# LuoGuiwen/MSM_blst

Measured on AMD Instinct MI355X. Metric: G1 MSM point-scalar pairs/sec at n=2^20, 1/2/4/8 MI355X; bit-exact vs CPU, higher is better.
Workload: dtype u32 (exact Fp381 integer arithmetic, 14x28-bit limbs)

## Files before the change

include/msm_mi355x.h:

```cpp
#ifndef MSM_MI355X_H
#define MSM_MI355X_H

#include <stddef.h>
#include <stdint.h>

#ifdef __cplusplus
extern "C" {
#endif

typedef uint8_t byte;
typedef uint64_t limb_t;
typedef struct { byte b[256 / 8]; } blst_scalar;
typedef struct { limb_t l[384 / 8 / sizeof(limb_t)]; } blst_fp;
typedef struct { blst_fp fp[2]; } blst_fp2;
typedef struct { blst_fp x, y, z; } blst_p1;
typedef struct { blst_fp x, y; } blst_p1_affine;
typedef struct { blst_fp2 x, y, z; } blst_p2;
typedef struct { blst_fp2 x, y; } blst_p2_affine;
typedef struct { blst_fp x, y, zzz, zz; } blst_p1xyzz;
typedef struct { blst_fp2 x, y, zzz, zz; } blst_p2xyzz;
typedef struct { int m; int b; int alpha; } digit_decomposition;

size_t blst_p1s_mult_pippenger_scratch_sizeof(size_t npoints);
void blst_p1s_mult_pippenger(blst_p1 *ret, const blst_p1_affine *const points[], size_t npoints,
// ... 222 lines not shown
void msm_gen_scalars(byte *out32, size_t n, uint64_t seed);
void msm_p1_fixed_points(blst_p1_affine *out, size_t n);
void msm_p2_fixed_points(blst_p2_affine *out, size_t n);
void msm_p1_fixed_points_range(blst_p1_affine *out, size_t start, size_t n);
void msm_p2_fixed_points_range(blst_p2_affine *out, size_t start, size_t n);
void msm_p1_to_affine(blst_p1_affine *out, const blst_p1 *in);
void msm_p2_to_affine(blst_p2_affine *out, const blst_p2 *in);
void msm_p1_compress(byte out[48], const blst_p1 *in);
void msm_p2_compress(byte out[96], const blst_p2 *in);
void msm_p1_add(blst_p1 *out, const blst_p1 *a, const blst_p1 *b);
void msm_p2_add(blst_p2 *out, const blst_p2 *a, const blst_p2 *b);

int msm_test_field(int group, int op, const limb_t *a, const limb_t *b, limb_t *out, size_t n);
int msm_test_xyzz(int group, const void *points_affine, size_t npoints, const uint32_t *ops, int len, size_t nseq,
                  void *out);

#ifdef __cplusplus
}
#endif
#endif
```

msm_blst_amd/_ffi.py:

```python
import ctypes
import os

HERE = os.path.dirname(os.path.abspath(__file__))
LIB_PATH = os.path.join(HERE, "libmsm_mi355x.so")

_lib = None


class MsmError(RuntimeError):
    pass


def lib():
    global _lib
    if _lib is not None:
        return _lib
    if not os.path.exists(LIB_PATH):
        raise MsmError(f"{LIB_PATH} not built: run `python -m msm_blst_amd.build` (hipcc, gfx950)")
    L = ctypes.CDLL(LIB_PATH)
    vp, sz, i32, u64 = ctypes.c_void_p, ctypes.c_size_t, ctypes.c_int, ctypes.c_uint64
    for g in (1, 2):
        f = getattr(L, f"blst_p{g}s_mult_pippenger")
        f.argtypes = [vp, vp, sz, vp, sz, vp]
        f.restype = None
# ... 9 lines not shown
            getattr(L, name).argtypes = [vp, vp]
        getattr(L, f"msm_p{g}_add").argtypes = [vp, vp, vp]
    L.msm_last_error.restype = ctypes.c_char_p
    L.msm_device_count.restype = i32
    L.msm_ctx_create.argtypes = [ctypes.POINTER(vp), i32, i32, i32]
    L.msm_ctx_set_points.argtypes = [vp, vp, sz, i32, vp]
    L.msm_ctx_mult.argtypes = [vp, vp, vp, sz, sz, i32, vp]
    L.msm_ctx_mult_batch.argtypes = [vp, vp, vp, sz, sz, sz, sz, i32, vp]
    L.msm_ctx_set_profiling.argtypes = [vp, i32]
    L.msm_ctx_phase_times.argtypes = [vp, vp]
    L.msm_ctx_destroy.argtypes = [vp]
    L.msm_ctx_destroy.restype = None
    L.msm_gen_scalars.argtypes = [vp, sz, u64]
    L.msm_test_field.argtypes = [i32, i32, vp, vp, vp, sz]
    L.msm_test_xyzz.argtypes = [i32, vp, sz, vp, i32, sz, vp]
    pp = ctypes.POINTER(vp)
    L.msm_ches_params.argtypes = [i32, i32, vp]
    L.msm_ches_ctx_create.argtypes = [pp, i32, i32, i32, i32]
    L.msm_ches_ctx_create_params.argtypes = [pp, i32, i32, vp]
    L.msm_ches_ctx_create_multi.argtypes = [pp, i32, vp, i32, i32, i32]
    L.msm_ches_ctx_shards.argtypes = [vp]
    L.msm_ches_ctx_build_table.argtypes = [vp, vp, sz, i32, vp]
    L.msm_ches_ctx_set_table.argtypes = [vp, vp, sz, i32, vp]
    L.msm_ches_ctx_get_table.argtypes = [vp, vp, sz, sz]
    L.msm_ches_ctx_mult.argtypes = [vp, vp, vp, sz, i32, vp]
    L.msm_ches_ctx_mult_batch.argtypes = [vp, vp, vp, sz, sz, sz, i32, vp]
    L.msm_ches_ctx_set_profiling.argtypes = [vp, i32]
    L.msm_ches_ctx_phase_times.argtypes = [vp, vp]
    L.msm_ches_ctx_bucket_count.argtypes = [vp]
    L.msm_ches_ctx_bucket_count.restype = sz
# ... 84 lines not shown
```

msm_blst_amd/csrc/abi.cpp:

```cpp
#include <hip/hip_runtime.h>
#include <stdio.h>
#include <stdlib.h>
#include <string.h>

#include <algorithm>
#include <atomic>
#include <map>
#include <memory>
#include <mutex>
#include <string>

#include "../../include/msm_mi355x.h"
#include "decode.hpp"
#include "encode.hpp"
#include "engine.hpp"
#include "hash_to_curve.hpp"
#include "multi.hpp"
#include "pairing.hpp"
#include "point_segments.hpp"
#include "points_mult.hpp"
#include "pool.hpp"
#include "ptr_walk.hpp"
#include "table_registry.hpp"
#include "to_affine.hpp"
// ... 1645 lines not shown
    return MSM_OK;
  } catch (const std::exception &e) {
    return fail(MSM_E_HIP, e.what());
  }
}
int msm_test_xyzz(int group, const void *pts, size_t npts, const uint32_t *ops, int len, size_t nseq, void *out) {
  try {
    if (group == 1) test_xyzz<1>((const uint64_t *)pts, npts, ops, len, nseq, (uint64_t *)out);
    else test_xyzz<2>((const uint64_t *)pts, npts, ops, len, nseq, (uint64_t *)out);
    return MSM_OK;
  } catch (const std::exception &e) {
    return fail(MSM_E_HIP, e.what());
  }
}

#define WB_DISPATCH(ctx, CALL) ((ctx)->group == 1 ? (ctx)->g1->CALL : (ctx)->g2->CALL)

int msm_wbits_ctx_create(msm_wbits_ctx **ctx, int group, int device, int wbits) {
  if (!ctx || (group != 1 && group != 2)) return fail(MSM_E_ARG, "bad ctx/group");
  if (msm_device_count() <= device || device < 0) return fail(MSM_E_NODEV, "no such HIP device");
  try {
    auto c = std::make_unique<msm_wbits_ctx>();
    c->group = group;
    c->device = device;
    if (group == 1) c->g1 = std::make_unique<Wbits<1>>(device, wbits);
    else c->g2 = std::make_unique<Wbits<2>>(device, wbits);
    *ctx = c.release();
    return MSM_OK;
  } catch (const std::exception &e) {
    return fail(MSM_E_ARG, e.what());
// ... 74 lines not shown
```

msm_blst_amd/csrc/bucket_sort.hpp:

```cpp
#pragma once
#include <hip/hip_runtime.h>
#include <stdint.h>

namespace msm {

constexpr int BS_TILE = 4096;
constexpr int BS_MAX_FB_BITS = 12;
constexpr int BS_MAX_CB = 8192;
constexpr uint32_t BS_NONE = 0xffffffffu;
constexpr int SCHED_PER_THREAD = 16;
constexpr int SCHED_PER_BLOCK = 256 * SCHED_PER_THREAD;
__device__ __forceinline__ uint32_t sched_class(uint32_t c) { return 255u - (c < 255u ? c : 255u); }

static __global__ void __launch_bounds__(256)
    k_bs_hist(const uint32_t *__restrict__ keys, size_t ne, int fb_bits, int ncb, int ntiles,
              uint32_t *__restrict__ ghist, uint32_t *__restrict__ classes) {
  __shared__ uint32_t h[BS_MAX_CB];
  keys += (size_t)blockIdx.y * ne;
  ghist += (size_t)blockIdx.y * ncb * ntiles;
  if (blockIdx.x == 0)
    for (int c = threadIdx.x; c < 512; c += blockDim.x) classes[(size_t)blockIdx.y * 512 + c] = 0;
  for (int b = threadIdx.x; b < ncb; b += blockDim.x) h[b] = 0;
  __syncthreads();
  const size_t t0 = (size_t)blockIdx.x * BS_TILE;
  uint32_t kk[BS_TILE / 256];
#pragma unroll
  for (int r = 0; r < BS_TILE / 256; ++r) {
    size_t e = t0 + threadIdx.x + (size_t)r * 256;
    kk[r] = e < ne ? keys[e] : BS_NONE;
  }
#pragma unroll
  for (int r = 0; r < BS_TILE / 256; ++r)
    if (kk[r] != BS_NONE) atomicAdd(&h[kk[r] >> fb_bits], 1u);
  __syncthreads();
  for (int b = threadIdx.x; b < ncb; b += blockDim.x) ghist[(size_t)b * ntiles + blockIdx.x] = h[b];
}

__device__ __forceinline__ uint32_t block_exclusive_scan_256(uint32_t *a, int n, uint32_t *wsum) {
  const int t = threadIdx.x, lane = t & 63, wave = t >> 6;
  const int per = (n + 255) / 256, lo = t * per, hi = min(n, lo + per);
  uint32_t s = 0;
  for (int i = lo; i < hi; ++i) s += a[i];
  uint32_t incl = s;
#pragma unroll
  for (int d = 1; d < 64; d <<= 1) {
    uint32_t v = __shfl_up(incl, d, 64);
    if (lane >= d) incl += v;
  }
  if (lane == 63) wsum[wave] = incl;
  __syncthreads();
// ... 92 lines not shown
    int i = t * per + k;
    if (k < per && i < n) a[i] = base + loc[k];
  }
  __syncthreads();
}

constexpr int BS_FINE_CAP = 30 * 1024;
constexpr int BS_FINE_STEP = BS_FINE_CAP - BS_FINE_CAP / 8;
constexpr int BS_FINE_MAXW = 8;

template <int BT>
static __global__ void __launch_bounds__(BT)
    k_bs_fine(const uint32_t *__restrict__ okeys, const uint32_t *__restrict__ ovals, int fb_bits, int ncb,
              int ntiles, const uint32_t *__restrict__ gbase, const uint32_t *__restrict__ ghist, uint32_t nb,
              uint32_t *__restrict__ sorted, uint32_t *__restrict__ counts, uint32_t *__restrict__ offsets,
              uint32_t *__restrict__ class_total, int nsets) {
  __shared__ uint32_t off[1 << BS_MAX_FB_BITS];
  __shared__ uint8_t win[1 << BS_MAX_FB_BITS];
  __shared__ uint32_t stage[BS_FINE_CAP];
  __shared__ uint32_t wsum[BT / 64];
  __shared__ uint32_t wb[BS_FINE_MAXW + 1];
  __shared__ uint32_t cls[256];
  const int FB = 1 << fb_bits;
  const uint32_t fmask = (uint32_t)FB - 1u;
  const int b = blockIdx.x, set = blockIdx.y;
  const size_t per = (size_t)ncb * ntiles, s0 = (size_t)set * per;
  const size_t last = (size_t)nsets * per - 1;
  const uint32_t lo = gbase[s0 + (size_t)b * ntiles];
  const uint32_t hi = b + 1 < ncb ? gbase[s0 + (size_t)(b + 1) * ntiles]
                                  : (set + 1 < nsets ? gbase[s0 + per] : gbase[last] + ghist[last]);
  counts += (size_t)set * nb;
  offsets += (size_t)set * nb;
  class_total += (size_t)set * 512;
  const uint32_t nbin = hi - lo;
  for (int f = threadIdx.x; f < FB; f += blockDim.x) off[f] = 0;
  for (int c = threadIdx.x; c < 256; c += BT) cls[c] = 0;
  if (threadIdx.x <= BS_FINE_MAXW) wb[threadIdx.x] = nbin;
  __syncthreads();
  constexpr int U = 16, UW = 12;
  for (uint32_t e0 = lo; e0 < hi; e0 += U * BT) {
    uint32_t kk[U];
#pragma unroll
    for (int r = 0; r < U; ++r) {
      uint32_t e = e0 + threadIdx.x + r * BT;
      kk[r] = e < hi ? okeys[e] : BS_NONE;
    }
#pragma unroll
    for (int r = 0; r < U; ++r)
      if (kk[r] != BS_NONE) atomicAdd(&off[kk[r] & fmask], 1u);
// ... 59 lines not shown
        if (kk[r] == BS_NONE || win[kk[r] & fmask] != k) continue;
        uint32_t li = atomicAdd(&off[kk[r] & fmask], 1u) - base;
        if (li < (uint32_t)BS_FINE_CAP)
          stage[li] = vv[r];
        else
          sorted[lo + base + li] = vv[r];
      }
    }
    __syncthreads();
    const uint32_t nst = min(end - base, (uint32_t)BS_FINE_CAP);
    for (uint32_t i = threadIdx.x; i < nst; i += BT) sorted[lo + base + i] = stage[i];
    __syncthreads();
  }
}

static __global__ void __launch_bounds__(256, 6)
    k_sched_scatter(const uint32_t *__restrict__ counts, const uint32_t *__restrict__ offsets, uint32_t nb,
                    uint32_t *__restrict__ class_total, uint32_t *__restrict__ order, uint32_t *__restrict__ scnt,
                    uint32_t *__restrict__ soff) {
  __shared__ uint32_t h[256];
  __shared__ uint32_t base[256];
  __shared__ uint32_t wsum[4];
  counts += (size_t)blockIdx.y * nb;
  offsets += (size_t)blockIdx.y * nb;
  order += (size_t)blockIdx.y * nb;
  scnt += (size_t)blockIdx.y * nb;
  soff += (size_t)blockIdx.y * nb;
  class_total += (size_t)blockIdx.y * 512;
  const uint32_t t = threadIdx.x, b0 = blockIdx.x * SCHED_PER_BLOCK, lane = t & 63, wave = t >> 6;
  h[t] = 0;
  const uint32_t v = class_total[t];
  uint32_t incl = v;
#pragma unroll
  for (int d = 1; d < 64; d <<= 1) {
    uint32_t u = __shfl_up(incl, d, 64);
    if (lane >= (uint32_t)d) incl += u;
  }
  if (lane == 63) wsum[wave] = incl;
  __syncthreads();
  uint32_t cbase = incl - v;
  for (uint32_t w = 0; w < wave; ++w) cbase += wsum[w];
  uint32_t rank[SCHED_PER_THREAD], cnt[SCHED_PER_THREAD];
#pragma unroll
  for (int r = 0; r < SCHED_PER_THREAD; ++r) {
    const uint32_t b = b0 + r * 256 + t;
    cnt[r] = b < nb ? counts[b] : 0u;
    rank[r] = b < nb ? atomicAdd(&h[sched_class(cnt[r])], 1u) : 0u;
  }
  __syncthreads();
  if (h[t]) base[t] = cbase + atomicAdd(&class_total[256 + t], h[t]);
  __syncthreads();
#pragma unroll
  for (int r = 0; r < SCHED_PER_THREAD; ++r) {
    const uint32_t b = b0 + r * 256 + t;
    if (b < nb) {
      const uint32_t pos = base[sched_class(cnt[r])] + rank[r];
      order[pos] = b;
      scnt[pos] = cnt[r];
      soff[pos] = offsets[b];
    }
  }
}

constexpr size_t BS_IPAY_SLACK = 64 * 256;
static __global__ void __launch_bounds__(256)
    k_interleave(const uint32_t *__restrict__ scnt, const uint32_t *__restrict__ soff, uint32_t nb, uint32_t nw,
                 const uint32_t *__restrict__ class_total, const uint32_t *__restrict__ sorted,
                 uint32_t *__restrict__ ipay, size_t ipay_stride, uint32_t *__restrict__ wbase) {
  __shared__ uint32_t ct[256], hs[256], wsum[4];
  const size_t set = blockIdx.y;
  const uint32_t t = threadIdx.x, lane = t & 63, wave = t >> 6;
  const uint32_t tot = class_total[set * 512 + t];
  uint32_t incl = tot;
// ... 53 lines not shown
```

msm_blst_amd/csrc/ches.hip:

```cpp
#include <hipcub/hipcub.hpp>

#include <algorithm>
#include <cstdlib>
#include <cstring>

#include "ches_kernels.hpp"
#include "coop.hpp"
#include "engine.hpp"
#include "hoststage.hpp"
#include "pair_kernels.hpp"

#ifndef MSM_GROUP
#error "define MSM_GROUP (1 or 2)"
#endif

namespace msm {

#if MSM_GROUP == 1
static const ChesParams kChesTable[] = {
    {8, 0, 12, 22, 7, 6, 857, 10, 26},         {9, 0, 13, 20, 231, 6, 1725, 11, 24},
    {10, 0, 13, 20, 231, 6, 1725, 12, 22},     {11, 0, 14, 19, 7, 6, 3417, 13, 20},
    {12, 0, 14, 19, 7, 6, 3417, 13, 20},       {13, 0, 16, 16, 29677, 6, 18343, 15, 17},
    {14, 0, 16, 16, 29677, 6, 18343, 15, 17},  {15, 0, 16, 16, 29677, 6, 18343, 16, 16},
    {16, 0, 19, 14, 231, 6, 109244, 17, 15},   {16, 1, 18, 15, 7, 6, 54618, 17, 15},
// ... 732 lines not shown
  f.counts.ensure(NB * nsets * 4);
  f.offsets.ensure(NB * nsets * 4);
  f.order.ensure(NB * nsets * 4);
  static const bool fused_env = [] {
    const char *e = getenv("MSM_FRONT_FUSED");
    return !e || atoi(e) != 0;
  }();
  if (fused_env && (p_.h == 12 || p_.h == 13 || p_.h == 14 || p_.h == 16 || p_.h == 19 || p_.h == 20)) {
    const int ntiles = (int)nblk(n, 256);
    const BucketSort::Geom g = f.sort.prepare(s, ne, (uint32_t)NB, nsets, ntiles);
#define MSM_CHES_FRONT(HT)                                                                                             \
  do {                                                                                                                 \
    hipLaunchKernelGGL(k_ches_front_hist<HT>, dim3(ntiles, nsets), dim3(256), 0, s, d_scalars, stride, n, p_.q_exp,   \
                       code_.as<uint32_t>(), rank_.as<uint2>(), (uint32_t)B_.size(), (uint32_t)small_,                 \
                       (uint32_t)copies_, set_stride, g.fb_bits, g.ncb, g.ntiles, f.sort.ghist.as<uint32_t>(),         \
                       f.sort.classes.as<uint32_t>());                                                                  \
    MSM_HIP_CHECK(hipGetLastError());                                                                                  \
    if (profile_) MSM_HIP_CHECK(hipEventRecord(ev_[1], s));                                                            \
    f.sort.scan(s, g);                                                                                                 \
    hipLaunchKernelGGL(k_ches_front_coarse<HT>, dim3(ntiles, nsets), dim3(256), (size_t)(2 * g.ncb + 512 * HT) * 4, s, \
                       d_scalars, stride, n, p_.q_exp, code_.as<uint32_t>(), rank_.as<uint2>(), (uint32_t)B_.size(),  \
                       (uint32_t)small_, (uint32_t)copies_, set_stride, g.fb_bits, g.ncb, g.ntiles,                   \
                       f.sort.gbase.as<uint32_t>(), f.sort.okeys.as<uint32_t>(), f.sort.ovals.as<uint32_t>());         \
    MSM_HIP_CHECK(hipGetLastError());                                                                                  \
  } while (0)
    switch (p_.h) {
      case 12: MSM_CHES_FRONT(12); break;
      case 13: MSM_CHES_FRONT(13); break;
      case 14: MSM_CHES_FRONT(14); break;
      case 16: MSM_CHES_FRONT(16); break;
      case 19: MSM_CHES_FRONT(19); break;
// ... 220 lines not shown
  }
  auto group_tail = [&](hipStream_t ts, int rset, size_t first, size_t nmsm, bool last_group) {
    if (bit_tail && last_group) {
      red.launch_tail_group_bits(ts, rset, (int)nmsm, tail_coop);
      red.copy_out_group_bits(ts, rset, (int)nmsm, host_bits_);
    } else {
      red.launch_tail_group(ts, rset, (int)nmsm, tail_coop && last_group);
      red.copy_out_group(ts, rset, (int)nmsm, out_base + first * ob);
    }
  };
  static const size_t fg_env = [] {
    const char *e = getenv("MSM_FRONT_GROUP");
    return e ? (size_t)std::min(kFrontGroup, std::max(1, atoi(e))) : (size_t)0;
  }();
  const int nl = batch_lanes();
  static const int fine_bt = [] {
    const char *e = getenv("MSM_FINE_BT");
    return e && atoi(e) == 256 ? 256 : 1024;
  }();
  static const bool acc_group_env = [] {
    const char *e = getenv("MSM_ACC_GROUP");
    return !e || atoi(e) != 0;
  }();
  const bool acc_groups = nl >= 2 && nseg == 1 && acc_group_env;
  const size_t fg_max = !packed ? 1 : fg_env ? fg_env : acc_groups ? 4 : nl >= 3 ? 4 : nl == 2 ? 2 : (size_t)kFrontGroupDefault;
  const std::vector<size_t> fgb = front_groups(count, fg_max);
  const size_t nfg = fgb.size() - 1;
  const size_t NB = bucket_count(), n = n_;
  if (acc_groups)
    for (DevBuf &b : gbuckets_) b.ensure(fg_max * NB * sizeof(Xyzz<typename FieldOf<G>::F>));
  else
    for (int b = 0; b < std::max(kBSets, nl); ++b) buckets_[b].ensure(NB * sizeof(Xyzz<typename FieldOf<G>::F>));
  static const bool phase_env = [] {
    const char *e = getenv("MSM_FRONT_PHASE");
// ... 286 lines not shown
```

msm_blst_amd/csrc/ches_kernels.hpp:

```cpp
#pragma once
#include "bucket_sort.hpp"
#include "kernels.hpp"

namespace msm {

constexpr uint32_t CH_IDX_MASK = 0x00ffffffu;

__device__ constexpr uint64_t PM2[6] = {0xb9feffffffffaaa9ull, 0x1eabfffeb153ffffull, 0x6730d2a0f6b0f624ull,
                                        0x64774b84f38512bfull, 0x4b1ba7b6434bacd7ull, 0x1a0111ea397fe69aull};
__device__ __forceinline__ void fp_inv(Fp &r, const Fp &a) {
  Fp a1 = a, a2, a3, acc;
  fp_norm(a1);
  fp_sqr(a2, a1);
  fp_mul(a3, a2, a1);
  fp_one(acc);
  for (int k = 190; k >= 0; --k) {
    if (k != 190) {
      fp_sqr(acc, acc);
      fp_sqr(acc, acc);
    }
    const uint32_t w = (uint32_t)(PM2[k >> 5] >> ((k & 31) * 2)) & 3u;
    if (w) {
      const uint32_t m1 = 0u - (uint32_t)(w == 1), m2 = 0u - (uint32_t)(w == 2), m3 = 0u - (uint32_t)(w == 3);
      Fp t;
// ... 270 lines not shown
    }
    if (j == HT - 1 && b != 0 && b <= small) {
      const uint32_t cp = (uint32_t)(i % copies);
      if (cp) b = nb0 + (cp - 1) * small + b - 1;
    }
    key[j] = b ? b : KEY_NONE;
    val[j] = (uint32_t)(3 * (i * (size_t)HT + j) + (c & 3u)) | ((c & 4u) << 29);
  }
}

template <int HT>
static __global__ void __launch_bounds__(256)
    k_ches_front_hist(const uint8_t *__restrict__ scalars, size_t stride, size_t n, int q_exp,
                      const uint32_t *__restrict__ code, const uint2 *__restrict__ rank, uint32_t nb0, uint32_t small,
                      uint32_t copies, size_t set_stride, int fb_bits, int ncb, int ntiles, uint32_t *__restrict__ ghist,
                      uint32_t *__restrict__ classes) {
  __shared__ uint32_t h[BS_MAX_CB];
  scalars += (size_t)blockIdx.y * set_stride;
  ghist += (size_t)blockIdx.y * ncb * ntiles;
  if (blockIdx.x == 0)
    for (int c = threadIdx.x; c < 512; c += blockDim.x) classes[(size_t)blockIdx.y * 512 + c] = 0;
  for (int b = threadIdx.x; b < ncb; b += blockDim.x) h[b] = 0;
  __syncthreads();
  const size_t i = (size_t)blockIdx.x * blockDim.x + threadIdx.x;
  if (i < n) {
    uint32_t key[HT], val[HT];
    ches_entries<HT>(scalars + i * stride, stride, i, q_exp, code, rank, nb0, small, copies, key, val);
#pragma unroll
    for (int j = 0; j < HT; ++j)
      if (key[j] != KEY_NONE) atomicAdd(&h[key[j] >> fb_bits], 1u);
  }
  __syncthreads();
  for (int b = threadIdx.x; b < ncb; b += blockDim.x) ghist[(size_t)b * ntiles + blockIdx.x] = h[b];
}

template <int HT>
static __global__ void __launch_bounds__(256)
    k_ches_front_coarse(const uint8_t *__restrict__ scalars, size_t stride, size_t n, int q_exp,
                        const uint32_t *__restrict__ code, const uint2 *__restrict__ rank, uint32_t nb0,
                        uint32_t small, uint32_t copies, size_t set_stride, int fb_bits, int ncb, int ntiles,
                        const uint32_t *__restrict__ gbase, uint32_t *__restrict__ okeys,
                        uint32_t *__restrict__ ovals) {
  extern __shared__ uint32_t sm[];
  __shared__ uint32_t wsum[4];
  uint32_t *loff = sm, *gb = sm + ncb, *sk = sm + 2 * ncb, *sv = sk + 256 * HT;
  scalars += (size_t)blockIdx.y * set_stride;
  gbase += (size_t)blockIdx.y * ncb * ntiles;
  for (int b = threadIdx.x; b < ncb; b += blockDim.x) {
    loff[b] = 0;
    gb[b] = gbase[(size_t)b * ntiles + blockIdx.x];
  }
  __syncthreads();
  const size_t i = (size_t)blockIdx.x * blockDim.x + threadIdx.x;
  uint32_t key[HT], val[HT], rk[HT];
  if (i < n) {
    ches_entries<HT>(scalars + i * stride, stride, i, q_exp, code, rank, nb0, small, copies, key, val);
  } else {
#pragma unroll
    for (int j = 0; j < HT; ++j) key[j] = KEY_NONE, val[j] = 0;
  }
#pragma unroll
  for (int j = 0; j < HT; ++j) rk[j] = key[j] != KEY_NONE ? atomicAdd(&loff[key[j] >> fb_bits], 1u) : 0u;
  __syncthreads();
  const uint32_t total = block_exclusive_scan_256(loff, ncb, wsum);
#pragma unroll
  for (int j = 0; j < HT; ++j) {
    if (key[j] == KEY_NONE) continue;
    const uint32_t pos = loff[key[j] >> fb_bits] + rk[j];
    sk[pos] = key[j];
    sv[pos] = val[j];
  }
  __syncthreads();
  for (uint32_t e = threadIdx.x; e < total; e += 256) {
    const uint32_t k = sk[e], b = k >> fb_bits;
    const uint32_t g = gb[b] + (e - loff[b]);
    okeys[g] = k;
    ovals[g] = sv[e];
  }
}

__device__ __forceinline__ void r_minus(uint32_t s[8]) {
  int64_t br = 0;
#pragma unroll
  for (int k = 0; k < 8; ++k) {
    int64_t d = (int64_t)FR_R32[k] - (int64_t)s[k] + br;
// ... 183 lines not shown
```

msm_blst_amd/csrc/engine.hip:

```cpp
#include <hipcub/hipcub.hpp>

#include <algorithm>

#include "bucket_sort.hpp"
#include "engine.hpp"
#include "hoststage.hpp"
#include "kernels.hpp"
#include "pair_kernels.hpp"

#ifndef MSM_GROUP
#error "define MSM_GROUP (1 or 2)"
#endif

namespace msm {

#if MSM_GROUP == 1
BucketSort::Geom BucketSort::prepare(hipStream_t s, size_t ne, uint32_t nb, int nsets, int ntiles) {
  Geom g;
  g.fb_bits = 8;
  while (g.fb_bits < BS_MAX_FB_BITS && ((size_t)nb >> g.fb_bits) > 384) ++g.fb_bits;
  g.ncb = (int)(((size_t)nb + (1u << g.fb_bits) - 1) >> g.fb_bits);
  if (g.ncb > BS_MAX_CB || g.ncb > 4096) throw std::runtime_error("BucketSort: too many buckets");
  if (nsets < 1 || nsets > 65535) throw std::runtime_error("BucketSort: bad set count");
  if (ne * nsets >= (1ull << 32)) throw std::runtime_error("BucketSort: too many entries");
  g.ntiles = ntiles > 0 ? ntiles : (int)std::max<size_t>(1, (ne + BS_TILE - 1) / BS_TILE);
  g.nslots = (size_t)nsets * g.ncb * g.ntiles;
  if (g.nslots >= (1ull << 31)) throw std::runtime_error("BucketSort: too many histogram slots");
  ghist.ensure(g.nslots * 4);
  gbase.ensure(g.nslots * 4);
  okeys.ensure(std::max<size_t>(ne * nsets, 1) * 4);
  ovals.ensure(std::max<size_t>(ne * nsets, 1) * 4);
  wbase.ensure(groups(nb) * nsets * 4);
  ipay_stride = ne + BS_IPAY_SLACK;
  ipay.ensure(ipay_stride * nsets * 4);
  size_t scan_tmp = 0;
  hipcub::DeviceScan::ExclusiveSum(nullptr, scan_tmp, ghist.as<uint32_t>(), gbase.as<uint32_t>(), (int)g.nslots, s);
  tmp.ensure(scan_tmp);
  g.scan_tmp = scan_tmp;
  classes.ensure((size_t)512 * 4 * nsets);
  scnt.ensure((size_t)nb * nsets * 4);
  soff.ensure((size_t)nb * nsets * 4);
  return g;
}

void BucketSort::scan(hipStream_t s, const Geom &g) {
  size_t tb = g.scan_tmp;
  MSM_HIP_CHECK(
      hipcub::DeviceScan::ExclusiveSum(tmp.p, tb, ghist.as<uint32_t>(), gbase.as<uint32_t>(), (int)g.nslots, s));
}

void BucketSort::run(hipStream_t s, const uint32_t *keys, const uint32_t *vals, size_t ne, uint32_t nb,
                     uint32_t *sorted, uint32_t *counts, uint32_t *offsets, uint32_t *order, int nsets) {
  const Geom g = prepare(s, ne, nb, nsets, 0);
  hipLaunchKernelGGL(k_bs_hist, dim3(g.ntiles, nsets), dim3(256), 0, s, keys, ne, g.fb_bits, g.ncb, g.ntiles,
                     ghist.as<uint32_t>(), classes.as<uint32_t>());
  MSM_HIP_CHECK(hipGetLastError());
  scan(s, g);
  hipLaunchKernelGGL(k_bs_coarse, dim3(g.ntiles, nsets), dim3(256), (size_t)(2 * g.ncb + 2 * BS_TILE) * 4, s, keys,
                     vals, ne, g.fb_bits, g.ncb, g.ntiles, gbase.as<uint32_t>(), okeys.as<uint32_t>(),
                     ovals.as<uint32_t>());
  MSM_HIP_CHECK(hipGetLastError());
  finish(s, g, ne, nb, sorted, counts, offsets, order, nsets);
}

void BucketSort::finish(hipStream_t s, const Geom &g, size_t ne, uint32_t nb, uint32_t *sorted, uint32_t *counts,
                        uint32_t *offsets, uint32_t *order, int nsets) {
  (void)ne;
  const int fb_bits = g.fb_bits, ncb = g.ncb, ntiles = g.ntiles;
  const size_t nw = groups(nb);
  if (fine_bt == 256)
    hipLaunchKernelGGL(k_bs_fine<256>, dim3(ncb, nsets), dim3(256), 0, s, okeys.as<uint32_t>(),
                       ovals.as<uint32_t>(), fb_bits, ncb, ntiles, gbase.as<uint32_t>(), ghist.as<uint32_t>(), nb,
                       sorted, counts, offsets, classes.as<uint32_t>(), nsets);
  else
    hipLaunchKernelGGL(k_bs_fine<1024>, dim3(ncb, nsets), dim3(1024), 0, s, okeys.as<uint32_t>(),
                       ovals.as<uint32_t>(), fb_bits, ncb, ntiles, gbase.as<uint32_t>(), ghist.as<uint32_t>(), nb,
                       sorted, counts, offsets, classes.as<uint32_t>(), nsets);
  MSM_HIP_CHECK(hipGetLastError());
  hipLaunchKernelGGL(k_sched_scatter, dim3(nblk(nb, SCHED_PER_BLOCK), nsets), dim3(256), 0, s, counts, offsets, nb,
                     classes.as<uint32_t>(), order, scnt.as<uint32_t>(), soff.as<uint32_t>());
  MSM_HIP_CHECK(hipGetLastError());
  hipLaunchKernelGGL(k_interleave, dim3((unsigned)nw / 4 + 1, nsets), dim3(256), 0, s, scnt.as<uint32_t>(),
                     soff.as<uint32_t>(), nb, (uint32_t)nw, classes.as<uint32_t>(), sorted, ipay.as<uint32_t>(),
                     ipay_stride, wbase.as<uint32_t>());
  MSM_HIP_CHECK(hipGetLastError());
}
#endif


template <int G>
Pippenger<G>::Pippenger(int device, int window_bits) : dev_(device), c_(window_bits) {
  if (c_ < 8 || c_ > 20) throw std::runtime_error("window_bits out of range [8,20]");
// ... 514 lines not shown
```

msm_blst_amd/csrc/engine.hpp:

```cpp
#pragma once
#include <hip/hip_runtime.h>
#include <stdint.h>

#include <cstdlib>
#include <memory>
#include <stdexcept>
#include <string>
#include <vector>

#include "acc_sched.hpp"
#include "host_fp.hpp"

#define MSM_HIP_CHECK(x)                                                                           \
  do {                                                                                            \
    hipError_t e_ = (x);                                                                          \
    if (e_ != hipSuccess)                                                                         \
      throw std::runtime_error(std::string("HIP error ") + hipGetErrorString(e_) + " at " + #x); \
  } while (0)

namespace msm {

class HostStager;

inline unsigned nblk(size_t n, unsigned b) { return (unsigned)((n + b - 1) / b); }
// ... 50 lines not shown
  int accumulate_launches = 0;
};

template <int G>
struct HostField;
template <>
struct HostField<1> {
  typedef hfp::Fp F;
};
template <>
struct HostField<2> {
  typedef hfp::Fp2 F;
};

struct BucketSort {
  DevBuf ghist, gbase, okeys, ovals, classes, tmp;
  DevBuf scnt, soff, wbase, ipay;
  size_t ipay_stride = 0;
  int fine_bt = 1024;
  static size_t groups(size_t nb) { return (nb + 63) / 64; }
  AccSched sched(const uint32_t *order, const uint32_t *sorted, size_t set, size_t nb) const {
    const size_t nw = groups(nb);
    return AccSched{order + set * nb,
                    scnt.as<uint32_t>() + set * nb,
                    soff.as<uint32_t>() + set * nb,
                    wbase.as<uint32_t>() + set * nw,
                    ipay.as<uint32_t>() + set * ipay_stride,
                    sorted};
  }
  AccStride stride(size_t nb) const { return AccStride{nb, groups(nb), ipay_stride}; }
  void run(hipStream_t s, const uint32_t *keys, const uint32_t *vals, size_t ne, uint32_t nb, uint32_t *sorted,
           uint32_t *counts, uint32_t *offsets, uint32_t *order, int nsets = 1);
  struct Geom {
    int fb_bits = 8, ncb = 1, ntiles = 1;
    size_t nslots = 0, scan_tmp = 0;
  };
  Geom prepare(hipStream_t s, size_t ne, uint32_t nb, int nsets, int ntiles);
  void scan(hipStream_t s, const Geom &g);
  void finish(hipStream_t s, const Geom &g, size_t ne, uint32_t nb, uint32_t *sorted, uint32_t *counts,
              uint32_t *offsets, uint32_t *order, int nsets);
  size_t device_bytes() const {
    return ghist.bytes + gbase.bytes + okeys.bytes + ovals.bytes + classes.bytes + tmp.bytes + scnt.bytes + soff.bytes +
           wbase.bytes + ipay.bytes;
  }
};

template <class HF>
hfp::Jac<HF> horner(const std::vector<hfp::Jac<HF>> &T, int c) {
  hfp::Jac<HF> ret = T.back();
  for (int w = (int)T.size() - 2; w >= 0; --w) {
    for (int k = 0; k < c; ++k) ret = hfp::dbl(ret);
    ret = hfp::addj(ret, T[w]);
  }
  return ret;
}


// ... 314 lines not shown
```

Baseline: 459.4 million.

## Replace hipcub scan with fused bin-total scan and add split fine-sort kernel

Drops the hipcub DeviceScan over the histogram. The histogram kernels now atomically accumulate per-bin totals, and a custom k_bs_scan kernel derives each bin's base from those totals and scans its tiles, so no temp buffer or multi-pass library scan is needed. The fine kernel resets bin_total so it can be reused on the next call. The change also adds an optional split fine-sort kernel, selected only via MSM_FINE_BT=split, compacts registers in the front-sort and sched-scatter kernels by packing rank and class bits, and adds a test entry point. The risks are atomic contention on bin_total and the quadratic prefix sum that each scan block does over earlier bins.

New measurement: 457.8 million. About the same (-0.3%).

```diff
diff --git a/include/msm_mi355x.h b/include/msm_mi355x.h
--- a/include/msm_mi355x.h
+++ b/include/msm_mi355x.h
@@ -260,6 +260,10 @@
 int msm_test_field(int group, int op, const limb_t *a, const limb_t *b, limb_t *out, size_t n);
 int msm_test_xyzz(int group, const void *points_affine, size_t npoints, const uint32_t *ops, int len, size_t nseq,
                   void *out);
+int msm_test_bucket_sort(int device, const uint32_t *d_keys, const uint32_t *d_vals, size_t ne, uint32_t nb, int nsets,
+                         int fine, uint32_t *counts, uint32_t *offsets, uint32_t *sorted, uint32_t *order,
+                         uint32_t *scnt, uint32_t *soff, uint32_t *wbase, uint32_t *ipay, uint32_t *ghist,
+                         uint32_t *gbase, size_t geom[4]);
 
 #ifdef __cplusplus
 }
diff --git a/msm_blst_amd/_ffi.py b/msm_blst_amd/_ffi.py
--- a/msm_blst_amd/_ffi.py
+++ b/msm_blst_amd/_ffi.py
@@ -47,6 +47,8 @@
     L.msm_gen_scalars.argtypes = [vp, sz, u64]
     L.msm_test_field.argtypes = [i32, i32, vp, vp, vp, sz]
     L.msm_test_xyzz.argtypes = [i32, vp, sz, vp, i32, sz, vp]
+    if hasattr(L, "msm_test_bucket_sort"):
+        L.msm_test_bucket_sort.argtypes = [i32, vp, vp, sz, ctypes.c_uint32, i32, i32] + [vp] * 11
     pp = ctypes.POINTER(vp)
     L.msm_ches_params.argtypes = [i32, i32, vp]
     L.msm_ches_ctx_create.argtypes = [pp, i32, i32, i32, i32]
diff --git a/msm_blst_amd/csrc/abi.cpp b/msm_blst_amd/csrc/abi.cpp
--- a/msm_blst_amd/csrc/abi.cpp
+++ b/msm_blst_amd/csrc/abi.cpp
@@ -1683,6 +1683,48 @@
   }
 }
 
+int msm_test_bucket_sort(int device, const uint32_t *d_keys, const uint32_t *d_vals, size_t ne, uint32_t nb, int nsets,
+                         int fine, uint32_t *counts, uint32_t *offsets, uint32_t *sorted, uint32_t *order,
+                         uint32_t *scnt, uint32_t *soff, uint32_t *wbase, uint32_t *ipay, uint32_t *ghist,
+                         uint32_t *gbase, size_t geom[4]) {
+  if (!d_keys || !d_vals || !ne || !nb || nsets < 1 || (fine != 1024 && fine != 256 && fine != BucketSort::FINE_SPLIT))
+    return fail(MSM_E_ARG, "bad args");
+  if (msm_device_count() <= device || device < 0) return fail(MSM_E_NODEV, "no such HIP device");
+  try {
+    DeviceGuard dg(device);
+    BucketSort bs;
+    bs.fine_bt = fine;
+    DevBuf d_sorted, d_counts, d_offsets, d_order;
+    const size_t nbs = (size_t)nb * nsets * 4;
+    d_sorted.ensure(ne * nsets * 4 + 64);
+    d_counts.ensure(nbs);
+    d_offsets.ensure(nbs);
+    d_order.ensure(nbs);
+    hipStream_t s = nullptr;
+    bs.run(s, d_keys, d_vals, ne, nb, d_sorted.as<uint32_t>(), d_counts.as<uint32_t>(), d_offsets.as<uint32_t>(),
+           d_order.as<uint32_t>(), nsets);
+    const BucketSort::Geom g = bs.prepare(s, ne, nb, nsets, 0);
+    MSM_HIP_CHECK(hipStreamSynchronize(s));
+    auto get = [&](uint32_t *dst, const void *src, size_t bytes) {
+      if (dst) MSM_HIP_CHECK(hipMemcpy(dst, src, bytes, hipMemcpyDeviceToHost));
+    };
+    get(counts, d_counts.p, nbs);
+    get(offsets, d_offsets.p, nbs);
+    get(order, d_order.p, nbs);
+    get(sorted, d_sorted.p, ne * nsets * 4);
+    get(scnt, bs.scnt.p, nbs);
+    get(soff, bs.soff.p, nbs);
+    get(wbase, bs.wbase.p, BucketSort::groups(nb) * nsets * 4);
+    get(ipay, bs.ipay.p, bs.ipay_stride * nsets * 4);
+    get(ghist, bs.ghist.p, g.nslots * 4);
+    get(gbase, bs.gbase.p, g.nslots * 4);
+    if (geom) geom[0] = (size_t)g.fb_bits, geom[1] = (size_t)g.ncb, geom[2] = (size_t)g.ntiles, geom[3] = bs.ipay_stride;
+    return MSM_OK;
+  } catch (const std::exception &e) {
+    return fail(MSM_E_HIP, e.what());
+  }
+}
+
 #define WB_DISPATCH(ctx, CALL) ((ctx)->group == 1 ? (ctx)->g1->CALL : (ctx)->g2->CALL)
 
 int msm_wbits_ctx_create(msm_wbits_ctx **ctx, int group, int device, int wbits) {
diff --git a/msm_blst_amd/csrc/bucket_sort.hpp b/msm_blst_amd/csrc/bucket_sort.hpp
--- a/msm_blst_amd/csrc/bucket_sort.hpp
+++ b/msm_blst_amd/csrc/bucket_sort.hpp
@@ -12,9 +12,15 @@
 constexpr int SCHED_PER_BLOCK = 256 * SCHED_PER_THREAD;
 __device__ __forceinline__ uint32_t sched_class(uint32_t c) { return 255u - (c < 255u ? c : 255u); }
 
+constexpr int FRONT_ACC_WAVES = 3;
+constexpr int front_vgpr_alloc(int vgprs) { return (vgprs + 7) / 8 * 8; }
+constexpr int front_vgpr_free(int acc_vgprs) { return 512 - FRONT_ACC_WAVES * front_vgpr_alloc(acc_vgprs); }
+constexpr int FRONT_MAX_THREADS = 256;
+constexpr int FRONT_MAX_LDS = 80 * 1024;
+
 static __global__ void __launch_bounds__(256)
     k_bs_hist(const uint32_t *__restrict__ keys, size_t ne, int fb_bits, int ncb, int ntiles,
-              uint32_t *__restrict__ ghist, uint32_t *__restrict__ classes) {
+              uint32_t *__restrict__ ghist, uint32_t *__restrict__ classes, uint32_t *__restrict__ bin_total) {
   __shared__ uint32_t h[BS_MAX_CB];
   keys += (size_t)blockIdx.y * ne;
   ghist += (size_t)blockIdx.y * ncb * ntiles;
@@ -33,7 +39,61 @@
   for (int r = 0; r < BS_TILE / 256; ++r)
     if (kk[r] != BS_NONE) atomicAdd(&h[kk[r] >> fb_bits], 1u);
   __syncthreads();
-  for (int b = threadIdx.x; b < ncb; b += blockDim.x) ghist[(size_t)b * ntiles + blockIdx.x] = h[b];
+  bin_total += (size_t)blockIdx.y * ncb;
+  for (int b = threadIdx.x; b < ncb; b += blockDim.x) {
+    ghist[(size_t)b * ntiles + blockIdx.x] = h[b];
+    if (h[b]) atomicAdd(&bin_total[b], h[b]);
+  }
+}
+
+static __global__ void __launch_bounds__(256)
+    k_bs_scan(const uint32_t *__restrict__ ghist, const uint32_t *__restrict__ bin_total, int ncb, int ntiles,
+              uint32_t *__restrict__ gbase) {
+  __shared__ uint32_t wsum[4];
+  const int t = threadIdx.x, lane = t & 63, wave = t >> 6;
+  const size_t slot = (size_t)blockIdx.y * ncb + blockIdx.x;
+  uint32_t s = 0;
+  for (size_t i = t; i < slot; i += 256) s += bin_total[i];
+#pragma unroll
+  for (int d = 32; d; d >>= 1) s += __shfl_xor(s, d, 64);
+  if (lane == 0) wsum[wave] = s;
+  __syncthreads();
+  uint32_t run = wsum[0] + wsum[1] + wsum[2] + wsum[3];
+  __syncthreads();
+  ghist += slot * ntiles;
+  gbase += slot * ntiles;
+  constexpr int PER = 4;
+  for (int c0 = 0; c0 < ntiles; c0 += 256 * PER) {
+    const int i0 = c0 + t * PER;
+    uint32_t x[PER], sum = 0;
+#pragma unroll
+    for (int k = 0; k < PER; ++k) {
+      x[k] = i0 + k < ntiles ? ghist[i0 + k] : 0u;
+      sum += x[k];
+    }
+    uint32_t incl = sum;
+#pragma unroll
+    for (int d = 1; d < 64; d <<= 1) {
+      uint32_t v = __shfl_up(incl, d, 64);
+      if (lane >= d) incl += v;
+    }
+    if (lane == 63) wsum[wave] = incl;
+    __syncthreads();
+    uint32_t before = 0, total = 0;
+#pragma unroll
+    for (int w = 0; w < 4; ++w) {
+      before += w < wave ? wsum[w] : 0u;
+      total += wsum[w];
+    }
+    uint32_t o = run + before + incl - sum;
+#pragma unroll
+    for (int k = 0; k < PER; ++k) {
+      if (i0 + k < ntiles) gbase[i0 + k] = o;
+      o += x[k];
+    }
+    run += total;
+    __syncthreads();
+  }
 }
 
 __device__ __forceinline__ uint32_t block_exclusive_scan_256(uint32_t *a, int n, uint32_t *wsum) {
@@ -156,7 +216,7 @@
     k_bs_fine(const uint32_t *__restrict__ okeys, const uint32_t *__restrict__ ovals, int fb_bits, int ncb,
               int ntiles, const uint32_t *__restrict__ gbase, const uint32_t *__restrict__ ghist, uint32_t nb,
               uint32_t *__restrict__ sorted, uint32_t *__restrict__ counts, uint32_t *__restrict__ offsets,
-              uint32_t *__restrict__ class_total, int nsets) {
+              uint32_t *__restrict__ class_total, int nsets, uint32_t *__restrict__ bin_total) {
   __shared__ uint32_t off[1 << BS_MAX_FB_BITS];
   __shared__ uint8_t win[1 << BS_MAX_FB_BITS];
   __shared__ uint32_t stage[BS_FINE_CAP];
@@ -175,6 +235,7 @@
   offsets += (size_t)set * nb;
   class_total += (size_t)set * 512;
   const uint32_t nbin = hi - lo;
+  if (threadIdx.x == 0) bin_total[(size_t)set * ncb + b] = 0;
   for (int f = threadIdx.x; f < FB; f += blockDim.x) off[f] = 0;
   for (int c = threadIdx.x; c < 256; c += BT) cls[c] = 0;
   if (threadIdx.x <= BS_FINE_MAXW) wb[threadIdx.x] = nbin;
@@ -264,7 +325,149 @@
   }
 }
 
-static __global__ void __launch_bounds__(256, 6)
+constexpr int BS_SPLIT_FR_BITS = 10;
+constexpr int BS_SPLIT_FR = 1 << BS_SPLIT_FR_BITS;
+constexpr int BS_SPLIT_CAP = 14 * 1024 + 384;
+constexpr int BS_SPLIT_STEP = BS_SPLIT_CAP - 512;
+constexpr int BS_SPLIT_MAXW = 8;
+__host__ __device__ constexpr int bs_split_parts(int fb_bits) {
+  return fb_bits > BS_SPLIT_FR_BITS ? 1 << (fb_bits - BS_SPLIT_FR_BITS) : 1;
+}
+
+static __global__ void __launch_bounds__(256)
+    k_bs_fine_split(const uint32_t *__restrict__ okeys, const uint32_t *__restrict__ ovals, int fb_bits, int ncb,
+                    int ntiles, const uint32_t *__restrict__ gbase, const uint32_t *__restrict__ ghist, uint32_t nb,
+                    uint32_t *__restrict__ sorted, uint32_t *__restrict__ counts, uint32_t *__restrict__ offsets,
+                    uint32_t *__restrict__ class_total, int nsets, uint32_t *__restrict__ bin_total) {
+  constexpr int BT = 256;
+  __shared__ uint32_t off[BS_SPLIT_FR];
+  __shared__ uint8_t win[BS_SPLIT_FR];
+  __shared__ uint32_t stage[BS_SPLIT_CAP];
+  __shared__ uint32_t wsum[BT / 64];
+  __shared__ uint32_t wb[BS_SPLIT_MAXW + 1];
+  __shared__ uint32_t cls[256];
+  __shared__ uint32_t below_s;
+  const int S = bs_split_parts(fb_bits);
+  const int FB = 1 << fb_bits, FR = FB / S;
+  const uint32_t fmask = (uint32_t)FB - 1u;
+  const int b = blockIdx.x / S, r = blockIdx.x % S, set = blockIdx.y;
+  const uint32_t f0 = (uint32_t)(r * FR);
+  const size_t per = (size_t)ncb * ntiles, s0 = (size_t)set * per;
+  const size_t last = (size_t)nsets * per - 1;
+  const uint32_t lo = gbase[s0 + (size_t)b * ntiles];
+  const uint32_t hi = b + 1 < ncb ? gbase[s0 + (size_t)(b + 1) * ntiles]
+                                  : (set + 1 < nsets ? gbase[s0 + per] : gbase[last] + ghist[last]);
+  counts += (size_t)set * nb;
+  offsets += (size_t)set * nb;
+  class_total += (size_t)set * 512;
+  if (threadIdx.x == 0) {
+    below_s = 0;
+    if (r == 0) bin_total[(size_t)set * ncb + b] = 0;
+  }
+  for (int f = threadIdx.x; f < FR; f += BT) off[f] = 0;
+  cls[threadIdx.x] = 0;
+  __syncthreads();
+  constexpr int U = 16, UW = 8;
+  uint32_t nbelow = 0;
+  for (uint32_t e0 = lo; e0 < hi; e0 += U * BT) {
+    uint32_t kk[U];
+#pragma unroll
+    for (int q = 0; q < U; ++q) {
+      uint32_t e = e0 + threadIdx.x + q * BT;
+      kk[q] = e < hi ? okeys[e] : BS_NONE;
+    }
+#pragma unroll
+    for (int q = 0; q < U; ++q) {
+      if (kk[q] == BS_NONE) continue;
+      const uint32_t f = (kk[q] & fmask) - f0;
+      if (f < (uint32_t)FR)
+        atomicAdd(&off[f], 1u);
+      else if ((kk[q] & fmask) < f0)
+        ++nbelow;
+    }
+  }
+#pragma unroll
+  for (int d = 32; d; d >>= 1) nbelow += __shfl_xor(nbelow, d, 64);
+  if ((threadIdx.x & 63) == 0 && nbelow) atomicAdd(&below_s, nbelow);
+  __syncthreads();
+  const uint32_t lo_own = lo + below_s;
+  for (int f = threadIdx.x; f < FR; f += BT) {
+    uint32_t bucket = ((uint32_t)b << fb_bits) + f0 + f;
+    if (bucket < nb) {
+      counts[bucket] = off[f];
+      atomicAdd(&cls[sched_class(off[f])], 1u);
+    }
+  }
+  __syncthreads();
+  if (cls[threadIdx.x]) atomicAdd(&class_total[threadIdx.x], cls[threadIdx.x]);
+  const uint32_t nown = block_exclusive_scan_256(off, FR, wsum);
+  const uint32_t nwin = (nown + BS_SPLIT_STEP - 1) / BS_SPLIT_STEP;
+  const bool staged = nwin <= (uint32_t)BS_SPLIT_MAXW;
+  if (threadIdx.x <= BS_SPLIT_MAXW) wb[threadIdx.x] = nown;
+  __syncthreads();
+  for (int f = threadIdx.x; f < FR; f += BT) {
+    uint32_t bucket = ((uint32_t)b << fb_bits) + f0 + f;
+    if (bucket < nb) offsets[bucket] = lo_own + off[f];
+    if (staged) {
+      uint32_t w = off[f] / BS_SPLIT_STEP;
+      win[f] = (uint8_t)w;
+      atomicMin(&wb[w], off[f]);
+    }
+  }
+  __syncthreads();
+  if (nown == 0) return;
+  if (!staged) {
+    for (uint32_t e0 = lo; e0 < hi; e0 += UW * BT) {
+      uint32_t kk[UW], vv[UW];
+#pragma unroll
+      for (int q = 0; q < UW; ++q) {
+        uint32_t e = e0 + threadIdx.x + q * BT;
+        kk[q] = e < hi ? okeys[e] : BS_NONE;
+        vv[q] = e < hi ? ovals[e] : 0u;
+      }
+#pragma unroll
+      for (int q = 0; q < UW; ++q) {
+        const uint32_t f = (kk[q] & fmask) - f0;
+        if (kk[q] == BS_NONE || f >= (uint32_t)FR) continue;
+        uint32_t pos = atomicAdd(&off[f], 1u);
+        sorted[lo_own + pos] = vv[q];
+      }
+    }
+    return;
+  }
+  for (uint32_t k = 0; k < nwin; ++k) {
+    const uint32_t base = wb[k];
+    if (base == nown) continue;
+    uint32_t end = nown;
+    for (uint32_t j = k + 1; j < nwin; ++j)
+      if (wb[j] < end) end = wb[j];
+    for (uint32_t e0 = lo; e0 < hi; e0 += UW * BT) {
+      uint32_t kk[UW], vv[UW];
+#pragma unroll
+      for (int q = 0; q < UW; ++q) {
+        uint32_t e = e0 + threadIdx.x + q * BT;
+        kk[q] = e < hi ? okeys[e] : BS_NONE;
+        vv[q] = e < hi ? ovals[e] : 0u;
+      }
+#pragma unroll
+      for (int q = 0; q < UW; ++q) {
+        const uint32_t f = (kk[q] & fmask) - f0;
+        if (kk[q] == BS_NONE || f >= (uint32_t)FR || win[f] != k) continue;
+        uint32_t li = atomicAdd(&off[f], 1u) - base;
+        if (li < (uint32_t)BS_SPLIT_CAP)
+          stage[li] = vv[q];
+        else
+          sorted[lo_own + base + li] = vv[q];
+      }
+    }
+    __syncthreads();
+    const uint32_t nst = min(end - base, (uint32_t)BS_SPLIT_CAP);
+    for (uint32_t i = threadIdx.x; i < nst; i += BT) sorted[lo_own + base + i] = stage[i];
+    __syncthreads();
+  }
+}
+
+static __global__ void __launch_bounds__(256)
     k_sched_scatter(const uint32_t *__restrict__ counts, const uint32_t *__restrict__ offsets, uint32_t nb,
                     uint32_t *__restrict__ class_total, uint32_t *__restrict__ order, uint32_t *__restrict__ scnt,
                     uint32_t *__restrict__ soff) {
@@ -290,12 +493,12 @@
   __syncthreads();
   uint32_t cbase = incl - v;
   for (uint32_t w = 0; w < wave; ++w) cbase += wsum[w];
-  uint32_t rank[SCHED_PER_THREAD], cnt[SCHED_PER_THREAD];
+  uint32_t rc[SCHED_PER_THREAD];
 #pragma unroll
   for (int r = 0; r < SCHED_PER_THREAD; ++r) {
     const uint32_t b = b0 + r * 256 + t;
-    cnt[r] = b < nb ? counts[b] : 0u;
-    rank[r] = b < nb ? atomicAdd(&h[sched_class(cnt[r])], 1u) : 0u;
+    const uint32_t cl = sched_class(b < nb ? counts[b] : 0u);
+    rc[r] = b < nb ? atomicAdd(&h[cl], 1u) | (cl << 16) : 0u;
   }
   __syncthreads();
   if (h[t]) base[t] = cbase + atomicAdd(&class_total[256 + t], h[t]);
@@ -304,9 +507,9 @@
   for (int r = 0; r < SCHED_PER_THREAD; ++r) {
     const uint32_t b = b0 + r * 256 + t;
     if (b < nb) {
-      const uint32_t pos = base[sched_class(cnt[r])] + rank[r];
+      const uint32_t pos = base[rc[r] >> 16] + (rc[r] & 0xffffu);
       order[pos] = b;
-      scnt[pos] = cnt[r];
+      scnt[pos] = counts[b];
       soff[pos] = offsets[b];
     }
   }
diff --git a/msm_blst_amd/csrc/ches.hip b/msm_blst_amd/csrc/ches.hip
--- a/msm_blst_amd/csrc/ches.hip
+++ b/msm_blst_amd/csrc/ches.hip
@@ -1,4 +1,3 @@
-#include <hipcub/hipcub.hpp>
 
 #include <algorithm>
 #include <cstdlib>
@@ -770,7 +769,7 @@
     hipLaunchKernelGGL(k_ches_front_hist<HT>, dim3(ntiles, nsets), dim3(256), 0, s, d_scalars, stride, n, p_.q_exp,   \
                        code_.as<uint32_t>(), rank_.as<uint2>(), (uint32_t)B_.size(), (uint32_t)small_,                 \
                        (uint32_t)copies_, set_stride, g.fb_bits, g.ncb, g.ntiles, f.sort.ghist.as<uint32_t>(),         \
-                       f.sort.classes.as<uint32_t>());                                                                  \
+                       f.sort.classes.as<uint32_t>(), f.sort.bin_total.as<uint32_t>());                                 \
     MSM_HIP_CHECK(hipGetLastError());                                                                                  \
     if (profile_) MSM_HIP_CHECK(hipEventRecord(ev_[1], s));                                                            \
     f.sort.scan(s, g);                                                                                                 \
@@ -1021,10 +1020,13 @@
     return e ? (size_t)std::min(kFrontGroup, std::max(1, atoi(e))) : (size_t)0;
   }();
   const int nl = batch_lanes();
-  static const int fine_bt = [] {
+  static const int fine_env = [] {
     const char *e = getenv("MSM_FINE_BT");
-    return e && atoi(e) == 256 ? 256 : 1024;
-  }();
+    if (!e) return -1;
+    if (!strcmp(e, "split")) return BucketSort::FINE_SPLIT;
+    return atoi(e) == 256 ? 256 : 1024;
+  }();
+  const int fine_bt = fine_env >= 0 ? fine_env : 1024;
   static const bool acc_group_env = [] {
     const char *e = getenv("MSM_ACC_GROUP");
     return !e || atoi(e) != 0;
diff --git a/msm_blst_amd/csrc/ches_kernels.hpp b/msm_blst_amd/csrc/ches_kernels.hpp
--- a/msm_blst_amd/csrc/ches_kernels.hpp
+++ b/msm_blst_amd/csrc/ches_kernels.hpp
@@ -308,7 +308,7 @@
     k_ches_front_hist(const uint8_t *__restrict__ scalars, size_t stride, size_t n, int q_exp,
                       const uint32_t *__restrict__ code, const uint2 *__restrict__ rank, uint32_t nb0, uint32_t small,
                       uint32_t copies, size_t set_stride, int fb_bits, int ncb, int ntiles, uint32_t *__restrict__ ghist,
-                      uint32_t *__restrict__ classes) {
+                      uint32_t *__restrict__ classes, uint32_t *__restrict__ bin_total) {
   __shared__ uint32_t h[BS_MAX_CB];
   scalars += (size_t)blockIdx.y * set_stride;
   ghist += (size_t)blockIdx.y * ncb * ntiles;
@@ -325,7 +325,11 @@
       if (key[j] != KEY_NONE) atomicAdd(&h[key[j] >> fb_bits], 1u);
   }
   __syncthreads();
-  for (int b = threadIdx.x; b < ncb; b += blockDim.x) ghist[(size_t)b * ntiles + blockIdx.x] = h[b];
+  bin_total += (size_t)blockIdx.y * ncb;
+  for (int b = threadIdx.x; b < ncb; b += blockDim.x) {
+    ghist[(size_t)b * ntiles + blockIdx.x] = h[b];
+    if (h[b]) atomicAdd(&bin_total[b], h[b]);
+  }
 }
 
 template <int HT>
@@ -346,23 +350,37 @@
   }
   __syncthreads();
   const size_t i = (size_t)blockIdx.x * blockDim.x + threadIdx.x;
-  uint32_t key[HT], val[HT], rk[HT];
-  if (i < n) {
-    ches_entries<HT>(scalars + i * stride, stride, i, q_exp, code, rank, nb0, small, copies, key, val);
-  } else {
-#pragma unroll
-    for (int j = 0; j < HT; ++j) key[j] = KEY_NONE, val[j] = 0;
-  }
-#pragma unroll
-  for (int j = 0; j < HT; ++j) rk[j] = key[j] != KEY_NONE ? atomicAdd(&loff[key[j] >> fb_bits], 1u) : 0u;
+  uint32_t key[HT], rk[HT];
+  const uint32_t slot0 = (uint32_t)(3 * (i * (size_t)HT));
+  {
+    uint32_t val[HT];
+    if (i < n) {
+      ches_entries<HT>(scalars + i * stride, stride, i, q_exp, code, rank, nb0, small, copies, key, val);
+    } else {
+#pragma unroll
+      for (int j = 0; j < HT; ++j) key[j] = KEY_NONE, val[j] = 0;
+    }
+#pragma unroll
+    for (int j = 0; j < HT; ++j) {
+      const uint32_t r = key[j] != KEY_NONE ? atomicAdd(&loff[key[j] >> fb_bits], 1u) : 0u;
+      sk[j * 256 + threadIdx.x] = key[j];
+      sv[j * 256 + threadIdx.x] = r | (((val[j] - (slot0 + 3u * j)) & 3u) << 16) | ((val[j] >> 31) << 18);
+    }
+  }
   __syncthreads();
   const uint32_t total = block_exclusive_scan_256(loff, ncb, wsum);
 #pragma unroll
   for (int j = 0; j < HT; ++j) {
+    key[j] = sk[j * 256 + threadIdx.x];
+    rk[j] = sv[j * 256 + threadIdx.x];
+  }
+  __syncthreads();
+#pragma unroll
+  for (int j = 0; j < HT; ++j) {
     if (key[j] == KEY_NONE) continue;
-    const uint32_t pos = loff[key[j] >> fb_bits] + rk[j];
+    const uint32_t pos = loff[key[j] >> fb_bits] + (rk[j] & 0xffffu);
     sk[pos] = key[j];
-    sv[pos] = val[j];
+    sv[pos] = (slot0 + 3u * j + ((rk[j] >> 16) & 3u)) | ((rk[j] >> 18) << 31);
   }
   __syncthreads();
   for (uint32_t e = threadIdx.x; e < total; e += 256) {
diff --git a/msm_blst_amd/csrc/engine.hip b/msm_blst_amd/csrc/engine.hip
--- a/msm_blst_amd/csrc/engine.hip
+++ b/msm_blst_amd/csrc/engine.hip
@@ -1,5 +1,3 @@
-#include <hipcub/hipcub.hpp>
-
 #include <algorithm>
 
 #include "bucket_sort.hpp"
@@ -33,10 +31,10 @@
   wbase.ensure(groups(nb) * nsets * 4);
   ipay_stride = ne + BS_IPAY_SLACK;
   ipay.ensure(ipay_stride * nsets * 4);
-  size_t scan_tmp = 0;
-  hipcub::DeviceScan::ExclusiveSum(nullptr, scan_tmp, ghist.as<uint32_t>(), gbase.as<uint32_t>(), (int)g.nslots, s);
-  tmp.ensure(scan_tmp);
-  g.scan_tmp = scan_tmp;
+  if (bin_total.bytes < (size_t)nsets * g.ncb * 4) {
+    bin_total.ensure((size_t)nsets * g.ncb * 4);
+    MSM_HIP_CHECK(hipMemsetAsync(bin_total.p, 0, bin_total.bytes, s));
+  }
   classes.ensure((size_t)512 * 4 * nsets);
   scnt.ensure((size_t)nb * nsets * 4);
   soff.ensure((size_t)nb * nsets * 4);
@@ -44,16 +42,17 @@
 }
 
 void BucketSort::scan(hipStream_t s, const Geom &g) {
-  size_t tb = g.scan_tmp;
-  MSM_HIP_CHECK(
-      hipcub::DeviceScan::ExclusiveSum(tmp.p, tb, ghist.as<uint32_t>(), gbase.as<uint32_t>(), (int)g.nslots, s));
+  const int nsets = (int)(g.nslots / ((size_t)g.ncb * g.ntiles));
+  hipLaunchKernelGGL(k_bs_scan, dim3(g.ncb, nsets), dim3(256), 0, s, ghist.as<uint32_t>(), bin_total.as<uint32_t>(),
+                     g.ncb, g.ntiles, gbase.as<uint32_t>());
+  MSM_HIP_CHECK(hipGetLastError());
 }
 
 void BucketSort::run(hipStream_t s, const uint32_t *keys, const uint32_t *vals, size_t ne, uint32_t nb,
                      uint32_t *sorted, uint32_t *counts, uint32_t *offsets, uint32_t *order, int nsets) {
   const Geom g = prepare(s, ne, nb, nsets, 0);
   hipLaunchKernelGGL(k_bs_hist, dim3(g.ntiles, nsets), dim3(256), 0, s, keys, ne, g.fb_bits, g.ncb, g.ntiles,
-                     ghist.as<uint32_t>(), classes.as<uint32_t>());
+                     ghist.as<uint32_t>(), classes.as<uint32_t>(), bin_total.as<uint32_t>());
   MSM_HIP_CHECK(hipGetLastError());
   scan(s, g);
   hipLaunchKernelGGL(k_bs_coarse, dim3(g.ntiles, nsets), dim3(256), (size_t)(2 * g.ncb + 2 * BS_TILE) * 4, s, keys,
@@ -68,14 +67,19 @@
   (void)ne;
   const int fb_bits = g.fb_bits, ncb = g.ncb, ntiles = g.ntiles;
   const size_t nw = groups(nb);
-  if (fine_bt == 256)
+  if (fine_bt == FINE_SPLIT)
+    hipLaunchKernelGGL(k_bs_fine_split, dim3(ncb * bs_split_parts(fb_bits), nsets), dim3(256), 0, s,
+                       okeys.as<uint32_t>(), ovals.as<uint32_t>(), fb_bits, ncb, ntiles, gbase.as<uint32_t>(),
+                       ghist.as<uint32_t>(), nb, sorted, counts, offsets, classes.as<uint32_t>(), nsets,
+                       bin_total.as<uint32_t>());
+  else if (fine_bt == 256)
     hipLaunchKernelGGL(k_bs_fine<256>, dim3(ncb, nsets), dim3(256), 0, s, okeys.as<uint32_t>(),
                        ovals.as<uint32_t>(), fb_bits, ncb, ntiles, gbase.as<uint32_t>(), ghist.as<uint32_t>(), nb,
-                       sorted, counts, offsets, classes.as<uint32_t>(), nsets);
+                       sorted, counts, offsets, classes.as<uint32_t>(), nsets, bin_total.as<uint32_t>());
   else
     hipLaunchKernelGGL(k_bs_fine<1024>, dim3(ncb, nsets), dim3(1024), 0, s, okeys.as<uint32_t>(),
                        ovals.as<uint32_t>(), fb_bits, ncb, ntiles, gbase.as<uint32_t>(), ghist.as<uint32_t>(), nb,
-                       sorted, counts, offsets, classes.as<uint32_t>(), nsets);
+                       sorted, counts, offsets, classes.as<uint32_t>(), nsets, bin_total.as<uint32_t>());
   MSM_HIP_CHECK(hipGetLastError());
   hipLaunchKernelGGL(k_sched_scatter, dim3(nblk(nb, SCHED_PER_BLOCK), nsets), dim3(256), 0, s, counts, offsets, nb,
                      classes.as<uint32_t>(), order, scnt.as<uint32_t>(), soff.as<uint32_t>());
diff --git a/msm_blst_amd/csrc/engine.hpp b/msm_blst_amd/csrc/engine.hpp
--- a/msm_blst_amd/csrc/engine.hpp
+++ b/msm_blst_amd/csrc/engine.hpp
@@ -88,9 +88,11 @@
 };
 
 struct BucketSort {
-  DevBuf ghist, gbase, okeys, ovals, classes, tmp;
+  DevBuf ghist, gbase, okeys, ovals, classes;
+  DevBuf bin_total;
   DevBuf scnt, soff, wbase, ipay;
   size_t ipay_stride = 0;
+  static constexpr int FINE_SPLIT = 0;
   int fine_bt = 1024;
   static size_t groups(size_t nb) { return (nb + 63) / 64; }
   AccSched sched(const uint32_t *order, const uint32_t *sorted, size_t set, size_t nb) const {
@@ -107,14 +109,14 @@
            uint32_t *counts, uint32_t *offsets, uint32_t *order, int nsets = 1);
   struct Geom {
     int fb_bits = 8, ncb = 1, ntiles = 1;
-    size_t nslots = 0, scan_tmp = 0;
+    size_t nslots = 0;
   };
   Geom prepare(hipStream_t s, size_t ne, uint32_t nb, int nsets, int ntiles);
   void scan(hipStream_t s, const Geom &g);
   void finish(hipStream_t s, const Geom &g, size_t ne, uint32_t nb, uint32_t *sorted, uint32_t *counts,
               uint32_t *offsets, uint32_t *order, int nsets);
   size_t device_bytes() const {
-    return ghist.bytes + gbase.bytes + okeys.bytes + ovals.bytes + classes.bytes + tmp.bytes + scnt.bytes + soff.bytes +
+    return ghist.bytes + gbase.bytes + okeys.bytes + ovals.bytes + classes.bytes + bin_total.bytes + scnt.bytes + soff.bytes +
            wbase.bytes + ipay.bytes;
   }
 };
```
